# alexranaldi/CWSL_DIGI

Measured on AMD Instinct MI355X. Metric: IQ Msamples/s demod+sync per GPU; concurrent FT8 slots at real-time; % HBM roofline, higher is better.
Workload: dtype f32

## Files before the change

### cwsl_digi_amd/csrc/cwsl_gpu.hip

```cpp
#include <hip/hip_runtime.h>
#include <rccl/rccl.h>
#include <dlfcn.h>

#include <algorithm>
#include <atomic>
#include <cctype>
#include <chrono>
#include <condition_variable>
#include <cstdarg>
#include <cstdio>
#include <cstdlib>
#include <cstring>
#include <map>
#include <memory>
#include <mutex>
#include <shared_mutex>
#include <string>
#include <tuple>
#include <vector>

#ifndef CWSLG_LAB
#define CWSLG_LAB 0
#endif

// ... 123 lines not shown
    int64_t origin_abs = 0;
    bool use_priv = false;
    PhasorTable priv;
    bool trans_active = false;
    std::shared_ptr<TransWork> trans;
    int64_t pend_lo = 0;
    uint32_t pend_n = 0;
    uint64_t pend_fill0 = 0;
    bool saturated = false;
    bool have_frame = false;
    int frame_idx = 0;
    uint64_t frame_t0 = 0;
    size_t frame_valid = 0;
    bool fin_fused = false;
    FinWork fused_fin{};
    size_t i16_end = ~size_t(0);
    uint64_t cand_t0 = 0;
    SyncChannelBuffers syncbuf;
};

struct WorkBuf {
    void *h = nullptr;
    void *h_dev = nullptr;
    void *d = nullptr;
    size_t bytes = 0;
    hipEvent_t done = nullptr;
    bool in_flight = false;
};

struct TimedSpan {
    hipEvent_t a, b;
    int kind;
    unsigned gen;
};

}

using namespace cwslg;

struct cwslg_ctx {
    std::mutex mu;
    int device = 0;
    int cu_count = 256;
    int order_override = 0;
    bool exact = true;
    bool upload_by_dma = false;
    int demod_variant = 0;
    hipStream_t stream = nullptr;
    std::string last_error;
    std::mutex err_mu;
    float scale_ft = 0.90f, scale_wspr = 0.20f;
    std::vector<Receiver> rxs;
    std::vector<Channel> chans;
    std::map<uint32_t, float *> d_taps;
    std::map<uint32_t, float *> d_taps2;
    const char *demod_kernel_name = "";
    std::map<uint32_t, std::vector<float>> h_taps;
    std::map<std::tuple<uint32_t, int32_t, int, size_t>, PhasorTable> phasors;
    std::vector<decltype(phasors)::key_type> phasor_todo;
    float2 *d_sincos = nullptr;
    hipStream_t copy_stream[kCopyStreams] = {};
    hipEvent_t copy_done[kCopyStreams] = {};
    hipEvent_t demod_done = nullptr;
    bool copies_pending[kCopyStreams] = {};
    bool copy_on_main = true;
    hipStream_t fetch_stream[kFetchStreams] = {};
    hipEvent_t fetch_ev[CWSLG_NUM_GROUPS] = {};
    bool fetch_ev_valid[CWSLG_NUM_GROUPS] = {};
    unsigned fetch_rr = 0;
    std::mutex fetch_mu;
    std::condition_variable fetch_cv;
    int fetch_inflight[CWSLG_NUM_GROUPS] = {};
    std::shared_mutex life_mu;
    BatchStage batch[kBatchStages];
    std::atomic<unsigned> batch_next{0};
    std::atomic<uint64_t> push_calls_a{0}, push_host_ns_a{0};
    unsigned long long *clk_h = nullptr, *clk_dev = nullptr;
    unsigned clk_head = 0, clk_tail = 0;
    unsigned exact5_seg_cap = kExact5SegCap, exact5_seg_force = 0;
#ifndef CWSLG_FUSE_FIN_DEFAULT
#define CWSLG_FUSE_FIN_DEFAULT 1
#endif
#ifndef CWSLG_FUSE_MODE_DEFAULT
#define CWSLG_FUSE_MODE_DEFAULT 1
#endif
    int fuse_mode = CWSLG_FUSE_MODE_DEFAULT;
    bool fuse_finalize = CWSLG_FUSE_FIN_DEFAULT != 0;
    int process_min_outputs = 0;
    bool use_exact5 = true;
    unsigned stat_gen = 0;
    double clk_sum_mhz = 0.0;
    int occ_cache[3][5] = {};
    WorkBuf wb[kWorkBufs];
    int wb_next = 0;
    size_t wb_largest = 0;
    cwslg_stats stats{};
    bool timing = false;
    std::vector<TimedSpan> spans;
    std::vector<std::pair<hipEvent_t, hipEvent_t>> ev_pool;
    SyncConfig sync_cfg;
    SyncShared sync_shared;
    Ft4Tables ft4_tables{};
    bool ft4_dft_valu = false;
    LongConfig long_cfg;
    LongShared long_shared;
    hipStream_t side = nullptr;
    hipEvent_t sync2d_done = nullptr, cand_done = nullptr, sync_tail = nullptr;
    bool cand_pending = false;
    int long_variant = 0;
    int sync_variant = 0;
    cwslg_rendezvous_fn rdv_fn = nullptr;
    void *rdv_user = nullptr;
    ncclComm_t rccl_comm = nullptr;
    uint64_t *d_rdv = nullptr, *h_rdv = nullptr;
    int rccl_world = 0;
    std::atomic<uint64_t> rdv_flag{0}, rdv_flags_and{0};
    bool rdv_pending = false;
    int rdv_group = 0;
    uint64_t rdv_epoch = 0, rdv_mine = 0;
    hipEvent_t rdv_ready = nullptr;
};

namespace {

int fail(cwslg_ctx *c, int code, const char *fmt, ...)
{
    char buf[512];
    va_list ap;
    va_start(ap, fmt);
    vsnprintf(buf, sizeof(buf), fmt, ap);
    va_end(ap);
    if (c) {
        std::lock_guard<std::mutex> g(c->err_mu);
        c->last_error = buf;
    }
    return code;
}

#define HIPCHK(ctx, expr)                                                                        \
    do {                                                                                         \
        hipError_t e_ = (expr);                                                                  \
        if (e_ != hipSuccess)                                                                    \
            return fail(ctx, CWSLG_ERR_HIP, "%s failed: %s (%s:%d)", #expr, hipGetErrorString(e_), \
                        __FILE__, __LINE__);                                                     \
    } while (0)

int sync_launch(cwslg_ctx *c, const std::vector<int> &emitted);
int sync_ensure_channel(cwslg_ctx *c, Channel &ch);
int long_sync_launch(cwslg_ctx *c, const std::vector<int> &emitted);

WorkBuf *acquire_workbuf(cwslg_ctx *c, size_t bytes)
{
    WorkBuf &w = c->wb[c->wb_next];
    c->wb_next = (c->wb_next + 1) % kWorkBufs;
    if (w.in_flight) {
        hipEventSynchronize(w.done);
        w.in_flight = false;
    }
    if (w.bytes < bytes) {
        if (w.h) hipHostFree(w.h);
        if (w.d) hipFree(w.d);
        static_assert(sizeof(SyncWork) <= 128 && sizeof(ChanWork) <= 128 && sizeof(FinWork) <= 128, "per-channel descriptors");
        size_t nb = std::max<size_t>(std::max(std::max(bytes, c->wb_largest), c->chans.size() * (size_t)128), 64 << 10);
        nb = (nb + 4095) & ~size_t(4095);
        c->wb_largest = nb;
        if (hipHostMalloc(&w.h, nb, hipHostMallocDefault) != hipSuccess) return nullptr;
        if (hipHostGetDevicePointer(&w.h_dev, w.h, 0) != hipSuccess) w.h_dev = nullptr;
// ... 658 lines not shown
    }
    return CWSLG_OK;
}

int rendezvous_failed(cwslg_ctx *c, int rc)
{
    std::string inner;
    {
        std::lock_guard<std::mutex> g(c->err_mu);
        if (c->last_error.rfind("slot-boundary rendezvous:", 0) == 0) inner = c->last_error;
    }
    if (!inner.empty()) return fail(c, rc, "slot-boundary rendezvous failed (%d): %s", rc, inner.c_str() + sizeof("slot-boundary rendezvous:"));
    return fail(c, rc, "slot-boundary rendezvous failed (%d)", rc);
}

}

#include "sync_host.inc"
#include "multi_gpu.inc"
#include "longsync_host.inc"

extern "C" {

int cwslg_abi_version(void) { return CWSLG_ABI_VERSION; }

const char *cwslg_strerror(int s)
{
    switch (s) {
    case CWSLG_OK: return "ok";
    case CWSLG_ERR_RATIO: return "Fs/B must be an even integer >= 4";
    case CWSLG_ERR_BAND_LOW: return "Signal outside of band (low)";
    case CWSLG_ERR_BAND_HIGH: return "Signal outside of band (high)";
    case CWSLG_ERR_NOMEM: return "out of memory";
    case CWSLG_ERR_MODE: return "Unhandled mode";
    case CWSLG_ERR_ARG: return "invalid argument";
    case CWSLG_ERR_NO_DEVICE: return "no usable HIP device (gfx950 required; there is no CPU fallback)";
    case CWSLG_ERR_HIP: return "HIP runtime error";
    case CWSLG_ERR_NO_FRAME: return "no finalised frame";
    case CWSLG_ERR_UNSUPPORTED: return "unsupported sample rate";
    case CWSLG_ERR_BLOCK: return "block length must be a multiple of SSBD::GetInSize()";
    default: return "unknown status";
    }
}

const char *cwslg_last_error(cwslg_ctx *ctx)
{
    if (!ctx) return "";
    static thread_local std::string copy;
    std::lock_guard<std::mutex> g(ctx->err_mu);
    copy = ctx->last_error;
    return copy.c_str();
}

int cwslg_create(cwslg_ctx **out, int device_ordinal)
{
    if (!out) return CWSLG_ERR_ARG;
    *out = nullptr;
    int n = 0;
    if (hipGetDeviceCount(&n) != hipSuccess || n <= 0) return CWSLG_ERR_NO_DEVICE;
    if (device_ordinal < 0) {
        const char *lr = std::getenv("LOCAL_RANK");
        device_ordinal = lr ? std::atoi(lr) % n : 0;
    }
    if (device_ordinal >= n) return CWSLG_ERR_NO_DEVICE;
    if (hipSetDevice(device_ordinal) != hipSuccess) return CWSLG_ERR_NO_DEVICE;
    hipDeviceProp_t prop;
    if (hipGetDeviceProperties(&prop, device_ordinal) != hipSuccess) return CWSLG_ERR_NO_DEVICE;
    if (std::strncmp(prop.gcnArchName, "gfx950", 6) != 0) return CWSLG_ERR_NO_DEVICE;
    std::unique_ptr<cwslg_ctx, void (*)(cwslg_ctx *)> c(new cwslg_ctx, cwslg_destroy);
    c->device = device_ordinal;
    c->cu_count = prop.multiProcessorCount > 0 ? prop.multiProcessorCount : 256;
#if CWSLG_LAB
    if (const char *v = std::getenv("CWSLG_DEMOD_VARIANT")) c->demod_variant = std::atoi(v);
    if (c->demod_variant != 0) c->use_exact5 = false;
    if (const char *v = std::getenv("CWSLG_EXACT5_SEG")) c->exact5_seg_cap = (unsigned)std::max(4, std::atoi(v));
    if (const char *v = std::getenv("CWSLG_EXACT5_SEG_FORCE")) c->exact5_seg_force = (unsigned)std::max(4, std::atoi(v)) / 4 * 4;
    if (const char *v = std::getenv("CWSLG_UPLOAD")) c->upload_by_dma = std::strcmp(v, "dma") == 0;
    if (const char *v = std::getenv("CWSLG_FT4_DFT")) c->ft4_dft_valu = std::strcmp(v, "valu") == 0;
    if (const char *v = std::getenv("CWSLG_ITEM_ORDER")) c->order_override = std::atoi(v);
    if (const char *v = std::getenv("CWSLG_SYNC_VARIANT")) c->sync_variant = std::atoi(v);
    if (const char *v = std::getenv("CWSLG_LONG_VARIANT")) c->long_variant = std::atoi(v);
    if (const char *v = std::getenv("CWSLG_COPY_ON_MAIN")) c->copy_on_main = std::atoi(v) != 0;
    if (const char *v = std::getenv("CWSLG_FUSE_FIN")) c->fuse_finalize = std::atoi(v) != 0;
    if (const char *v = std::getenv("CWSLG_FUSE_MODE")) c->fuse_mode = std::atoi(v) == 2 ? 2 : 1;
#endif
    if (hipStreamCreateWithFlags(&c->stream, hipStreamNonBlocking) != hipSuccess) return CWSLG_ERR_HIP;
    for (int k = 0; k < kCopyStreams; ++k) {
        if (hipStreamCreateWithFlags(&c->copy_stream[k], hipStreamNonBlocking) != hipSuccess) return CWSLG_ERR_HIP;
        hipEventCreateWithFlags(&c->copy_done[k], hipEventDisableTiming);
    }
    hipEventCreateWithFlags(&c->demod_done, kOrderEvent);
    for (int k = 0; k < kFetchStreams; ++k)
        if (hipStreamCreateWithFlags(&c->fetch_stream[k], hipStreamNonBlocking) != hipSuccess) return CWSLG_ERR_HIP;
    for (hipEvent_t &e : c->fetch_ev) hipEventCreateWithFlags(&e, hipEventDisableTiming);
    if (hipStreamCreateWithFlags(&c->side, hipStreamNonBlocking) != hipSuccess) return CWSLG_ERR_HIP;
    hipEventCreateWithFlags(&c->sync2d_done, hipEventDisableTiming);
    hipEventCreateWithFlags(&c->cand_done, hipEventDisableTiming);
    hipEventCreateWithFlags(&c->sync_tail, hipEventDisableTiming);
    {
        std::vector<float2> tab(4096);
        constexpr double pi = 3.14159265358979323846;
        for (int j = 0; j < 4096; ++j)
            tab[j] = make_float2((float)std::cos(2.0 * pi * j / 4096.0), (float)std::sin(2.0 * pi * j / 4096.0));
        if (hipMalloc(&c->d_sincos, tab.size() * sizeof(float2)) != hipSuccess) return CWSLG_ERR_NOMEM;
        if (hipMemcpy(c->d_sincos, tab.data(), tab.size() * sizeof(float2), hipMemcpyHostToDevice) != hipSuccess) return CWSLG_ERR_HIP;
    }
    *out = c.release();
    return CWSLG_OK;
}

void cwslg_destroy(cwslg_ctx *c)
{
    if (!c) return;
    hipSetDevice(c->device);
    for (hipStream_t cs : c->copy_stream) if (cs) hipStreamSynchronize(cs);
    if (c->side) hipStreamSynchronize(c->side);
    if (c->stream) hipStreamSynchronize(c->stream);
    for (hipStream_t fs : c->fetch_stream) if (fs) (void)hipStreamSynchronize(fs);
    for (Channel &ch : c->chans) {
        if (ch.d_block) hipFree(ch.d_block);
        sync_free_channel(ch.syncbuf);
        if (ch.longbuf.d_block) { (void)hipFree(ch.longbuf.d_block); ch.longbuf = LongChannelBuffers(); }
        if (ch.priv.d_ckpt) { (void)hipFree(ch.priv.d_ckpt); ch.priv.d_ckpt = nullptr; }
    }
    for (Receiver &rx : c->rxs) if (rx.d_ring) hipFree(rx.d_ring);
    for (auto &kv : c->d_taps) hipFree(kv.second);
    for (auto &kv : c->d_taps2) hipFree(kv.second);
    for (auto &kv : c->phasors) if (kv.second.d_ckpt) hipFree(kv.second.d_ckpt);
    for (WorkBuf &w : c->wb) {
        if (w.h) hipHostFree(w.h);
        if (w.d) hipFree(w.d);
        if (w.done) hipEventDestroy(w.done);
    }
    drain_spans(c);
    for (auto &p : c->ev_pool) { hipEventDestroy(p.first); hipEventDestroy(p.second); }
    rccl_release(c);
    sync_free_shared(c->sync_shared);
    long_free_shared(c->long_shared);
    if (c->d_sincos) hipFree(c->d_sincos);
    if (c->clk_h) (void)hipHostFree(c->clk_h);
    for (hipStream_t fs : c->fetch_stream) if (fs) { (void)hipStreamSynchronize(fs); (void)hipStreamDestroy(fs); }
    for (hipEvent_t e : c->fetch_ev) if (e) (void)hipEventDestroy(e);
    for (BatchStage &b : c->batch) {
        if (b.h) (void)hipHostFree(b.h);
        if (b.ev) (void)hipEventDestroy(b.ev);
    }
    for (int k = 0; k < kCopyStreams; ++k) {
        if (c->copy_stream[k]) { hipStreamSynchronize(c->copy_stream[k]); hipStreamDestroy(c->copy_stream[k]); }
        if (c->copy_done[k]) hipEventDestroy(c->copy_done[k]);
    }
    if (c->demod_done) hipEventDestroy(c->demod_done);
    if (c->rdv_ready) hipEventDestroy(c->rdv_ready);
    if (c->side) { hipStreamSynchronize(c->side); hipStreamDestroy(c->side); }
    for (hipEvent_t e : {c->sync2d_done, c->cand_done, c->sync_tail}) if (e) hipEventDestroy(e);
    if (c->stream) hipStreamDestroy(c->stream);
    delete c;
}

int cwslg_set_scale_factors(cwslg_ctx *c, float ft, float wspr)
{
    if (!c) return CWSLG_ERR_ARG;
    std::lock_guard<std::mutex> g(c->mu);
    c->scale_ft = ft;
    c->scale_wspr = wspr;
    return CWSLG_OK;
}

// ... 1124 lines not shown
```

### cwsl_digi_amd/csrc/sync_host.inc

```
namespace {

int sync_ensure_shared(cwslg_ctx *c)
{
    if (c->sync_shared.d_tables) return CWSLG_OK;
    constexpr double pi = 3.14159265358979323846;
    auto w = [&](int k, double n) { return make_float2((float)std::cos(2.0 * pi * k / n), (float)(-std::sin(2.0 * pi * k / n))); };
    auto half = [](float2 v) { return make_float2(0.5f * v.x, 0.5f * v.y); };
    auto same = [](float a, float b) { return std::memcmp(&a, &b, 4) == 0; };
    for (int k = 1; k <= 4; ++k)
        if (!same(w(k, 9.0).x, small_wr<9>(k)) || !same(w(k, 9.0).y, small_wi<9>(k)))
            return fail(c, CWSLG_ERR_HIP, "sync tables: W_9^%d computed on this host differs from the kernels' constants", k);
    for (int k = 1; k <= 2; ++k)
        if (!same(w(k, 5.0).x, w5_r(k)) || !same(w(k, 5.0).y, w5_i(k)))
            return fail(c, CWSLG_ERR_HIP, "sync tables: W_5^%d computed on this host differs from the kernels' constants", k);
    if (!same((float)(-std::sin(2.0 * pi / 3.0)), W3_S))
        return fail(c, CWSLG_ERR_HIP, "sync tables: sin(2 pi / 3) computed on this host differs from the kernels' constant");
    std::vector<float2> t;
    t.reserve(1920 + 64 + 1921 + 1152 + 1153);
    const float fac = 1.0f / 300.0f;
    for (int k = 0; k < 1920; ++k) { const float2 v = (k == 0) ? make_float2(1.f, 0.f) : w(k, 1920.0); t.push_back(make_float2(fac * v.x, fac * v.y)); }
    for (int k = 0; k < 64; ++k) t.push_back(w(k, 128.0));
    for (int k = 0; k <= 1920; ++k) t.push_back(half(k == 0 ? make_float2(1.f, 0.f) : w(k, 3840.0)));
    t[1920] = make_float2(1.f, 0.f); t[1920 + 32] = make_float2(0.f, -1.f);
    const size_t ft8_count = t.size();
// ... 124 lines not shown
int sync_launch(cwslg_ctx *c, const std::vector<int> &emitted)
{
    int rc = sync_ensure_shared(c);
    if (rc) return rc;
    const SyncConfig &cfg = c->sync_cfg;
    std::vector<SyncWork> works8, works4;
    std::vector<Ft4Work> works4c;
    for (int id : emitted) {
        Channel &ch = c->chans[id];
        if (!ch.sync_ft8 && !ch.sync_ft4) continue;
        rc = sync_ensure_channel(c, ch);
        if (rc) return rc;
        SyncWork w{};
        w.frame = ch.d_i16;
        w.spectra = ch.syncbuf.d_spectra;
        w.red = ch.syncbuf.d_red; w.red2 = ch.syncbuf.d_red2;
        w.jpeak = ch.syncbuf.d_jpeak; w.jpeak2 = ch.syncbuf.d_jpeak2;
        w.cand = ch.syncbuf.d_cand; w.ncand = ch.syncbuf.d_ncand;
        if (ch.fin_fused) { w.fin = ch.fused_fin; ch.fin_fused = false; }
        (ch.sync_ft8 ? works8 : works4).push_back(w);
        ch.cand_t0 = ch.frame_t0;
        if (ch.sync_ft4 && cfg.ft4_coherent) {
            if ((rc = ft4c_ensure_tables(c)) != CWSLG_OK || (rc = ft4c_ensure_channel(c, ch)) != CWSLG_OK) return rc;
            Ft4Work f{};
            f.frame = ch.d_i16; f.y = ch.syncbuf.d_y; f.cx = ch.syncbuf.d_cx;
            f.cand = ch.syncbuf.d_cand; f.ncand = ch.syncbuf.d_ncand;
            f.rec = (Ft4Rec *)ch.syncbuf.d_rec; f.nrec = ch.syncbuf.d_nrec; f.cd_dbg = ch.syncbuf.d_cd_dbg;
            works4c.push_back(f);
        }
    }
    if (works8.empty() && works4.empty()) return CWSLG_OK;
    const size_t n8 = works8.size(), n4 = works4.size();
    WorkBuf *wb = acquire_workbuf(c, (n8 + n4) * sizeof(SyncWork));
    if (!wb) return fail(c, CWSLG_ERR_NOMEM, "work buffer allocation failed");
    if (n8) std::memcpy(wb->h, works8.data(), n8 * sizeof(SyncWork));
    if (n4) std::memcpy((SyncWork *)wb->h + n8, works4.data(), n4 * sizeof(SyncWork));
    HIPCHK(c, upload_workbuf(c, wb, (n8 + n4) * sizeof(SyncWork)));
    WorkBuf *wb4 = nullptr;
    if (!works4c.empty()) {
        wb4 = acquire_workbuf(c, works4c.size() * sizeof(Ft4Work));
        if (!wb4) return fail(c, CWSLG_ERR_NOMEM, "work buffer allocation failed");
        std::memcpy(wb4->h, works4c.data(), works4c.size() * sizeof(Ft4Work));
        HIPCHK(c, upload_workbuf(c, wb4, works4c.size() * sizeof(Ft4Work)));
    }
    hipEvent_t ea, eb;
    const bool chain_async = n8 && !n4 && (c->sync_variant & 32);
    const bool cand_async = n8 && (c->sync_variant & 8) && !chain_async;
    if (n8 && c->cand_pending) {
        HIPCHK(c, hipStreamWaitEvent(c->stream, c->cand_done, 0));
        c->cand_pending = false;
    }
    hipStream_t s8 = c->stream;
    if (chain_async) {
        s8 = c->side;
        HIPCHK(c, hipEventRecord(c->sync2d_done, c->stream));
        HIPCHK(c, hipStreamWaitEvent(c->side, c->sync2d_done, 0));
        span_begin_on(c, 2, c->side, &ea, &eb);
    } else {
        span_begin(c, 2, &ea, &eb);
    }
    if (n8) {
        const SyncWork *d8 = (const SyncWork *)wb->d;
        const unsigned nbands = (unsigned)((cfg.ib - cfg.ia + 1 + SYNC_BAND - 1) / SYNC_BAND);
#if CWSLG_LAB
        if (c->sync_variant & 2)
            hipLaunchKernelGGL((symbol_spectra_kernel<15, FT8_NSPS, FT8_NSTEP, false>), dim3(FT8_NHSYM, (unsigned)n8), dim3(256), 0,
                               s8, d8, c->sync_shared.t, cfg.nbins);
        else
#endif
        {
        hipEvent_t pa = nullptr, pb = nullptr;
        if (s8 == c->stream) span_begin(c, 3, &pa, &pb);
        const int jper8 = spectra_jper(FT8_NHSYM, n8);
        bool fused8 = works8[0].fin.frame != nullptr;
        for (const SyncWork &sw : works8) if ((sw.fin.frame != nullptr) != fused8) return fail(c, CWSLG_ERR_ARG, "mixed fused / separate finalise in one launch");
        const dim3 g8((FT8_NHSYM + jper8 - 1) / jper8, (unsigned)n8);
        if (!fused8) {
#if CWSLG_LAB || !CWSLG_FUSE_FIN_DEFAULT
            hipLaunchKernelGGL((symbol_spectra_v2_kernel<15, FT8_NSPS, FT8_NSTEP, false, 0>), g8, dim3(256), 0, s8, d8, c->sync_shared.t, cfg.nbins, FT8_NHSYM, jper8);
#else
            return fail(c, CWSLG_ERR_ARG, "FT8 frame reached the sync stage without its finalise");
#endif
        }
#if CWSLG_LAB || CWSLG_FUSE_MODE_DEFAULT == 2
        else if (c->fuse_mode == 2)
            hipLaunchKernelGGL((symbol_spectra_v2_kernel<15, FT8_NSPS, FT8_NSTEP, false, 2>), g8, dim3(256), 0, s8, d8, c->sync_shared.t, cfg.nbins, FT8_NHSYM, jper8);
#endif
        else
            hipLaunchKernelGGL((symbol_spectra_v2_kernel<15, FT8_NSPS, FT8_NSTEP, false, 1>), g8, dim3(256), 0, s8, d8, c->sync_shared.t, cfg.nbins, FT8_NHSYM, jper8);
        span_end(c, pb);
        }
        const bool per_channel = n8 >= (size_t)2 * (size_t)c->cu_count;
#if CWSLG_LAB
        if (!(c->sync_variant & (1 | 64 | 128))) {
#endif
        hipEvent_t qa = nullptr, qb = nullptr;
        if (s8 == c->stream) span_begin(c, 4, &qa, &qb);
        if (per_channel) {
            hipLaunchKernelGGL(ft8_sync_chan_kernel, dim3((unsigned)n8), dim3(SYNCC_NT), 0, s8, d8, cfg.ia, cfg.ib, cfg.nbins, cfg.syncmin, cfg.max_cand, cfg.order);
        } else {
            hipLaunchKernelGGL(ft8_sync2d_v3_kernel, dim3(nbands, (unsigned)n8), dim3(SYNC2D_NT), 0, s8, d8, cfg.ia, cfg.ib, cfg.nbins);
            hipLaunchKernelGGL(ft8_candidates_kernel<1024>, dim3((unsigned)n8), dim3(1024), 0, s8, d8, cfg.ia, cfg.ib, cfg.syncmin, cfg.max_cand, cfg.order);
        }
        span_end(c, qb);
#if CWSLG_LAB
        } else {
        if (c->sync_variant & 1)
            hipLaunchKernelGGL(ft8_sync2d_kernel, dim3(nbands, (unsigned)n8), dim3(SYNC2D_NT), 0, s8, d8, cfg.ia, cfg.ib, cfg.nbins);
        else if (c->sync_variant & 64)
            hipLaunchKernelGGL(ft8_sync2d_v2_kernel, dim3(nbands, (unsigned)n8), dim3(SYNC2D_NT), 0, s8, d8, cfg.ia, cfg.ib, cfg.nbins);
        else
            hipLaunchKernelGGL(ft8_sync2d_v3_kernel, dim3(nbands, (unsigned)n8), dim3(SYNC2D_NT), 0, s8, d8, cfg.ia, cfg.ib, cfg.nbins);
        hipStream_t cs = s8;
        hipEvent_t sa = nullptr, sb = nullptr;
        if (cand_async) {
            cs = c->side;
            HIPCHK(c, hipEventRecord(c->sync2d_done, c->stream));
            HIPCHK(c, hipStreamWaitEvent(c->side, c->sync2d_done, 0));
            span_begin_on(c, 2, c->side, &sa, &sb);
        }
        if (c->sync_variant & 4)
            hipLaunchKernelGGL(ft8_candidates_kernel<256>, dim3((unsigned)n8), dim3(256), 0, cs, d8, cfg.ia, cfg.ib,
                               cfg.syncmin, cfg.max_cand, cfg.order);
        else
            hipLaunchKernelGGL(ft8_candidates_kernel<1024>, dim3((unsigned)n8), dim3(1024), 0, cs, d8, cfg.ia, cfg.ib,
                               cfg.syncmin, cfg.max_cand, cfg.order);
        if (cand_async) {
            if (sb) hipEventRecord(sb, c->side);
            HIPCHK(c, hipEventRecord(c->cand_done, c->side));
            c->cand_pending = true;
        }
        }
#endif
    }
    if (n4) {
        const SyncWork *d4 = (const SyncWork *)wb->d + n8;
        const float df4 = 12000.0f / (float)FT4_NFFT1;
        int nfa = (int)((float)cfg.f_lo_hz / df4), nfb = (int)((float)cfg.f_hi_hz / df4);
        nfa = std::max(nfa, (int)std::lround(200.0f / df4));
        nfb = std::min(nfb, (int)std::lround(4910.0f / df4));
        const int jper4 = spectra_jper(FT4_NHSYM, n4);
#if CWSLG_LAB
        if (c->sync_variant & 2)
            hipLaunchKernelGGL((symbol_spectra_kernel<9, FT4_NFFT1, FT4_NSTEP, true>), dim3(FT4_NHSYM, (unsigned)n4), dim3(256), 0,
                               c->stream, d4, c->sync_shared.t4, FT4_ROW);
        else
#endif
        hipLaunchKernelGGL((symbol_spectra_v2_kernel<9, FT4_NFFT1, FT4_NSTEP, true>), dim3((FT4_NHSYM + jper4 - 1) / jper4, (unsigned)n4), dim3(256), 0,
                           c->stream, d4, c->sync_shared.t4, FT4_ROW, FT4_NHSYM, jper4);
        hipLaunchKernelGGL(ft4_candidates_kernel, dim3((unsigned)n4), dim3(256), 0, c->stream, d4, nfa, nfb,
                           c->sync_cfg.syncmin_ft4, cfg.max_cand, cfg.order);
        if (c->sync_cfg.ft4_coherent) {
            const Ft4Work *f4 = (const Ft4Work *)wb4->d;
#if CWSLG_LAB
            if (c->ft4_dft_valu)
                hipLaunchKernelGGL(ft4_dft567_kernel, dim3((F4C_NA + 4 * F4C_CPT - 1) / (4 * F4C_CPT), (unsigned)n4), dim3(256), 0, c->stream, f4, c->ft4_tables);
            else
#endif
            hipLaunchKernelGGL(ft4_dft567_mfma_kernel, dim3(9, (unsigned)n4), dim3(256), 0, c->stream, f4, c->ft4_tables);
            hipLaunchKernelGGL(ft4_fft64_unpack_kernel, dim3(284, (unsigned)n4), dim3(64), 0, c->stream, f4, c->ft4_tables);
            hipLaunchKernelGGL(ft4_refine_kernel, dim3((unsigned)cfg.max_cand, (unsigned)n4), dim3(256), 0, c->stream, f4, c->ft4_tables, cfg.max_cand);
        }
    }
    if (chain_async) {
        if (eb) hipEventRecord(eb, c->side);
        HIPCHK(c, hipEventRecord(c->cand_done, c->side));
        c->cand_pending = true;
        HIPCHK(c, hipGetLastError());
        HIPCHK(c, hipEventRecord(wb->done, c->side));
        wb->in_flight = true;
        c->stats.sync_launches++;
        return CWSLG_OK;
// ... 175 lines not shown
```

### cwsl_digi_amd/csrc/sync_kernels.hpp

```cpp
#pragma once
#include <hip/hip_runtime.h>
#include <stdint.h>

namespace cwslg {

constexpr int FT8_NSPS = 1920, FT8_NSTEP = 480, FT8_NHSYM = 372, FT8_NH1 = 1920, FT8_JZ = 62, FT8_NMAX = 180000;
constexpr int FT4_NFFT1 = 2304, FT4_NSTEP = 576, FT4_NHSYM = 122, FT4_NH1 = 1152, FT4_NMAX = 72576;
constexpr int FT4_ROW = 1168;
constexpr int SYNC_BAND = 32;
constexpr int SYNC_MAXCAND_CAP = 600;
constexpr int SYNC_MAXPRE = 1000;

struct SyncConfig {
    bool enabled = false;
    float syncmin = 1.5f;
    float syncmin_ft4 = 1.2f;
    bool ft4_coherent = true;
    int max_cand = 200;
    int order = 0;
    int f_lo_hz = 200, f_hi_hz = 3000;
    int ia = 64, ib = 960, nbins = 976;
};

struct SyncTables {
// ... 391 lines not shown
#define CWSLG_SPEC_TIGHT 1
#endif
#ifndef CWSLG_PLANE_NT
#define CWSLG_PLANE_NT 0
#endif
__device__ __forceinline__ void plane_store(CWSLG_GLOBAL v4f *p, v4f v)
{
    if (CWSLG_PLANE_NT & 1) __builtin_nontemporal_store(v, p); else *p = v;
}
__device__ __forceinline__ v4f plane_load4(const CWSLG_GLOBAL v4f *p)
{
    return (CWSLG_PLANE_NT & 2) ? __builtin_nontemporal_load(p) : *p;
}
__device__ __forceinline__ float plane_load1(const CWSLG_GLOBAL float *p)
{
    return (CWSLG_PLANE_NT & 2) ? __builtin_nontemporal_load(p) : *p;
}
inline int spectra_jper(int nsteps, size_t channels)
{
    for (int jper : {62, 31}) if (channels * (size_t)((nsteps + jper - 1) / jper) >= 3072) return jper;
    return 12;
}
#if defined(CWSLG_STAMP) && defined(CWSLG_STAMP_SPEC)
#define PSTAMP(slot)                                                                                                               \
    do {                                                                                                                           \
        const unsigned wg_ = blockIdx.y * gridDim.x + blockIdx.x;                                                                  \
        if (j == j0 + (jper >> 1) && (tid_ & 63) == 0 && wg_ < 16384) {                                                                     \
            unsigned long long t_;                                                                                                 \
            asm volatile("s_memtime %0\n\ts_waitcnt lgkmcnt(0)" : "=s"(t_)::"memory");                                             \
            g_stamps[32 * wg_ + 8 * (tid_ >> 6) + (slot)] = t_;                                                                    \
        }                                                                                                                          \
    } while (0)
#else
#define PSTAMP(slot) do { } while (0)
#endif
struct SpectraFin {
    const CWSLG_GLOBAL float *frame;
    CWSLG_GLOBAL int16_t *out;
    unsigned nv, s_end;
    float factor;
};
__device__ __forceinline__ unsigned fin_pack2(float x0, float x1, float factor)
{
    const float s0 = x0 * factor, s1 = x1 * factor;
    const float b0 = s0 + 0.5f, b1 = s1 + 0.5f;
    const int q0 = (int)b0, q1 = (int)b1;
    return ((unsigned)q0 & 0xFFFFu) | ((unsigned)q1 << 16);
}
__device__ __forceinline__ void spectra_finalize_range(const SpectraFin &F, unsigned s0, unsigned s1)
{
    typedef unsigned v4u __attribute__((ext_vector_type(4)));
    constexpr int NC = 4;
    for (unsigned base = s0 + threadIdx.x * 8u; base < s1; base += 256u * 8u * (unsigned)NC) {
        v4f a[NC], b[NC];
#pragma unroll
        for (int c = 0; c < NC; ++c) {
            const unsigned i0 = base + (unsigned)c * (256u * 8u);
            if (i0 + 8 <= F.nv && i0 < s1) {
                a[c] = *reinterpret_cast<const CWSLG_GLOBAL v4f *>(F.frame + i0);
                b[c] = *reinterpret_cast<const CWSLG_GLOBAL v4f *>(F.frame + i0 + 4);
            } else {
                float v[8];
#pragma unroll
                for (int k = 0; k < 8; ++k) v[k] = (i0 + k < F.nv && i0 < s1) ? F.frame[i0 + k] : 0.0f;
                a[c] = v4f{v[0], v[1], v[2], v[3]};
                b[c] = v4f{v[4], v[5], v[6], v[7]};
            }
        }
#pragma unroll
        for (int c = 0; c < NC; ++c) {
            const unsigned i0 = base + (unsigned)c * (256u * 8u);
            if (i0 >= s1) break;
            v4u pk;
            pk.x = fin_pack2(a[c].x, a[c].y, F.factor); pk.y = fin_pack2(a[c].z, a[c].w, F.factor);
            pk.z = fin_pack2(b[c].x, b[c].y, F.factor); pk.w = fin_pack2(b[c].z, b[c].w, F.factor);
            *reinterpret_cast<CWSLG_GLOBAL v4u *>(F.out + i0) = pk;
        }
    }
}

template <int NA, int NIN, int STEP, bool WINDOW, int FMODE = 0>
__global__ __launch_bounds__(256, CWSLG_SPEC_WAVES) void symbol_spectra_v2_kernel(const SyncWork *__restrict__ works, SyncTables tb, int nbins, int nsteps, int jper)
{
    static_assert(FMODE == 0 || (!WINDOW && NIN == 4 * STEP && STEP == 480), "the fused forms are FT8's");
    constexpr int NZ = NA * 128;
    constexpr int NPACK = NIN / 2;
    constexpr int NGRP = NA * 16;
    constexpr int AMAX = (NPACK + 127) / 128;
    constexpr int NH = NA / 2;
    constexpr int NITEM = (NH + 1) * 64, IPT = (NITEM + 255) / 256;
    static_assert(NGRP <= 256, "geometry");
    __shared__ __attribute__((aligned(16))) float s_pw[NIN + 32];
    __shared__ float2 s_y[NA][SY_PITCH];
    __shared__ float2 s_w128[64];
    constexpr int RING = NPACK + STEP / 2;
    __shared__ unsigned s_ring[FMODE == 2 ? 2 * RING : 1];
    const SyncWork *w = works + blockIdx.y;
    const int j0 = blockIdx.x * jper;
    const int jend = min(j0 + jper, nsteps);
    const int tid_ = threadIdx.x;
    const int b_ = tid_ & 127;
    const float fac = 1.0f / 300.0f;
    const CWSLG_GLOBAL unsigned *d32 = as_global(reinterpret_cast<const unsigned *>(w->frame)) + b_;
    float *const plane = w->spectra;
    const bool fuse = FMODE != 0;
    SpectraFin F{};
    v2f cv = {0.0f, 0.0f};
    unsigned fin_i = ~0u;
    unsigned fin_lim = 0u;
    constexpr int LOOK = 3;
    unsigned ring_rd = 0u, ring_wr = 0u;
    if (fuse) {
        const FinWork &f = w->fin;
        F.frame = as_global(f.frame); F.out = as_global_rw(f.out); F.nv = f.n_valid;
        const unsigned flen = f.frame_len;
        const float peak = __uint_as_float(*as_global(f.peak));
        float factor = 32767.0f / (peak + 1.0f);
        factor = factor * f.scale;
        F.factor = factor;
        if (blockIdx.x == 0 && tid_ == 0) {
            if (f.peak_next) *as_global_rw(f.peak_next) = 0u;
            if (f.factor_out) *as_global_rw(f.factor_out) = factor;
        }
        const unsigned cover = min((unsigned)(STEP * (nsteps - 1) + NIN), flen), tail_end = min(max(f.tail_end, cover), flen);
        if (tail_end > cover) {
            const unsigned per = ((tail_end - cover + gridDim.x - 1) / gridDim.x + 7u) & ~7u;
            spectra_finalize_range(F, min(cover + per * blockIdx.x, tail_end), min(cover + per * (blockIdx.x + 1), tail_end));
        }
        if constexpr (FMODE == 1) {
            F.s_end = min(((unsigned)(STEP * (jend - 1) + NIN) + 63u) & ~63u, flen);
            const unsigned e0 = min(((unsigned)(STEP * (j0 + LOOK - 1) + NIN) + 63u) & ~63u, F.s_end);
            spectra_finalize_range(F, (unsigned)(STEP * j0) & ~63u, e0);
            __builtin_amdgcn_s_waitcnt(0x0F70);
            __syncthreads();
            fin_lim = min(F.nv & ~1u, F.s_end);
            fin_i = e0 + 2u * (unsigned)tid_;
        } else {
            F.s_end = min((unsigned)(STEP * (jend - 1) + NIN), flen);
            fin_lim = min(F.nv & ~1u, F.s_end);
            const unsigned p0 = (unsigned)(STEP / 2) * (unsigned)j0;
            for (unsigned k = (unsigned)tid_; k < (unsigned)NPACK; k += 256u) {
                const unsigned i = 2u * (p0 + k);
                v2f p = {0.0f, 0.0f};
                if (i < fin_lim) p = *reinterpret_cast<const CWSLG_GLOBAL v2f *>(F.frame + i);
                const v2f bi = p * F.factor + 0.5f;
                const unsigned word = __builtin_amdgcn_perm((unsigned)(int)bi.y, (unsigned)(int)bi.x, 0x05040100u);
                if (i < F.s_end) *reinterpret_cast<CWSLG_GLOBAL unsigned *>(F.out + i) = word;
                const unsigned pos = (p0 + k) % (unsigned)RING;
                s_ring[pos] = word; s_ring[pos + RING] = word;
            }
            __syncthreads();
            fin_i = tid_ < STEP / 2 ? (unsigned)(STEP * j0 + NIN) + 2u * (unsigned)tid_ : 0x40000000u;
            ring_rd = (p0 + (unsigned)b_) % (unsigned)RING;
            ring_wr = (p0 + (unsigned)NPACK + (unsigned)tid_) % (unsigned)RING;
        }
        if (fin_i < fin_lim) cv = *reinterpret_cast<const CWSLG_GLOBAL v2f *>(F.frame + fin_i);
    }
    unsigned raw[AMAX];
    if constexpr (FMODE != 2) {
#pragma unroll
        for (int a = 0; a < AMAX; ++a) raw[a] = (128 * a + b_ < NPACK) ? d32[(STEP / 2) * j0 + 128 * a] : 0u;
    } else {
#pragma unroll
        for (int a = 0; a < AMAX; ++a) raw[a] = s_ring[ring_rd + 128 * a];
        ring_rd += (unsigned)(STEP / 2); if (ring_rd >= (unsigned)RING) ring_rd -= (unsigned)RING;
    }
    float2 wn[WINDOW ? AMAX : 1];
    if (WINDOW) {
#pragma unroll
        for (int a = 0; a < AMAX; ++a) {
            const int m = 128 * a + b_;
            wn[WINDOW ? a : 0] = *reinterpret_cast<const float2 *>(tb.win + 2 * ((m < NPACK) ? m : 0));
        }
    }
    Stage1Tw<NA> tw1;
    if (tid_ < 128) stage1_load_tw<0, NA>(tb.w1920, b_, tw1);
    else stage1_load_tw<1, NA>(tb.w1920, b_, tw1);
    const bool sparse = nbins >= NA * 64 && nbins <= NA * 64 + 32 && NH == 7;
    constexpr unsigned PW_DUMMY = 4u * (NIN + 31);
    float2 w3[IPT][2];
#ifndef CWSLG_SPEC_UNHOIST
#define CWSLG_SPEC_UNHOIST 0
#endif
    struct ItemAddr { unsigned au1[IPT], au2[IPT], aw1[IPT], aw2[IPT], ap1[IPT], ap2[IPT], aB[8]; bool iskip[IPT], izero[IPT]; };
    auto item_addr = [&](int tidx, ItemAddr &A, int (&K1o)[IPT], int (&K2o)[IPT]) {
#pragma unroll
    for (int i = 0; i < IPT; ++i) {
        const int it = tidx + 256 * i;
        int r = it >> 6, q = it & 63, kind = 0;
        bool skip = it >= NITEM || (r == 0 && q > 32);
        int Kup = 0;
        if (sparse && i == 0 && r == 0 && q > 32) {
            Kup = NA * 64 - 32 + q;
            const int d = Kup - NA * 64, a = d / NA, rem = d % NA;
            if (rem <= NH) { kind = 2; r = rem; q = a; }
            else { kind = 3; r = NA - rem; q = 63 - a; }
            skip = Kup >= nbins;
        }
        const int r2 = (r == 0) ? 0 : NA - r;
        const int k2 = (r == 0) ? ((64 - q) & 63) : 63 - q;
        A.izero[i] = r == 0 && q == 0 && kind == 0;
        if (sparse && A.izero[i]) kind = 1;
        A.iskip[i] = skip;
        const int rr = skip ? 0 : r, rr2 = skip ? 0 : r2;
        static_assert((SY_PITCH * 8) % 128 == 0, "row pitch");
        A.au1[i] = 8u * (unsigned)(rr * SY_PITCH + sy_col(q));
        A.au2[i] = 8u * (unsigned)(rr2 * SY_PITCH + sy_col(k2));
        A.aw1[i] = 8u * (unsigned)q; A.aw2[i] = 8u * (unsigned)k2;
        int K1 = NA * q + r, K2 = NA * k2 + r2;
        unsigned p1 = 4u * (unsigned)K1, p2 = 4u * (unsigned)K2;
        if (kind == 1) { K2 = NA * 64; p2 = (K2 < nbins) ? 4u * (unsigned)K2 : PW_DUMMY; }
        if (kind >= 2) { K1 = Kup; p1 = 4u * (unsigned)Kup; K2 = nbins; p2 = PW_DUMMY; }
        A.ap1[i] = p1 | ((unsigned)kind << 16); A.ap2[i] = p2;
        K1o[i] = (!skip && K1 < nbins) ? K1 : -1; K2o[i] = (!skip && K2 < nbins) ? K2 : -1;
    }
    {
        const int c = tidx >> 4, g = tidx & 15, blk = g >> 3, r = g & 7;
#pragma unroll
        for (int q = 0; q < 8; ++q) A.aB[q] = 8u * (unsigned)((tidx < NGRP ? c : 0) * SY_PITCH + sy_col(64 * blk + r + 8 * q));
    }
    };
    ItemAddr IA0;
    {
        int K1o[IPT], K2o[IPT];
        item_addr(tid_, IA0, K1o, K2o);
#pragma unroll
        for (int i = 0; i < IPT; ++i) {
            w3[i][0] = K1o[i] >= 0 ? tb.w3840[K1o[i]] : make_float2(0.f, 0.f);
            w3[i][1] = K2o[i] >= 0 ? tb.w3840[K2o[i]] : make_float2(0.f, 0.f);
        }
    }
    const bool wave0_ = __builtin_amdgcn_readfirstlane(tid_ >> 6) == 0;
    if (tid_ >= 64 && tid_ < 128) s_w128[tid_ - 64] = tb.w128[tid_ - 64];
    __builtin_amdgcn_s_waitcnt(0x0F70);

    for (int j = j0; j < jend; ++j) {
    int t = tid_;
    asm volatile("" : "+v"(t));
    const int tid = t, b = t & 127;
    ItemAddr IAj;
    int k1j[IPT], k2j[IPT];
    if (CWSLG_SPEC_UNHOIST) item_addr(tid, IAj, k1j, k2j);
    const ItemAddr &IA = CWSLG_SPEC_UNHOIST ? IAj : IA0;
    char *const sy_bytes = reinterpret_cast<char *>(&s_y[0][0]);
    const char *const w128_bytes = reinterpret_cast<const char *>(&s_w128[0]);
    char *const pw_bytes = reinterpret_cast<char *>(&s_pw[0]);
    PSTAMP(0);
    float2 z[AMAX];
#pragma unroll
    for (int a = 0; a < AMAX; ++a) {
        const bool live = 128 * a + b < NPACK;
        float lo = (float)(short)(raw[a] & 0xFFFFu), hi = (float)(short)(raw[a] >> 16);
        if (NA != 15) { lo = fac * lo; hi = fac * hi; }
        if (WINDOW) { lo = lo * wn[WINDOW ? a : 0].x; hi = hi * wn[WINDOW ? a : 0].y; }
        z[a] = live ? make_float2(lo, hi) : make_float2(0.f, 0.f);
    }
#ifndef CWSLG_SPEC_LOADS_FIRST
#define CWSLG_SPEC_LOADS_FIRST 0
#endif
#ifndef CWSLG_FUSE_STORE_NT
#define CWSLG_FUSE_STORE_NT 0
#endif
    auto store_prev_row = [&]() {
#ifdef CWSLG_SPEC_DIAG_NOSTORE
        if (j > j0 && nbins < 0) {
#else
        if (j > j0) {
#endif
            CWSLG_GLOBAL v4f *out4 = reinterpret_cast<CWSLG_GLOBAL v4f *>(as_global_rw(CWSLG_SPEC_HOISTPTR ? plane : w->spectra) + (size_t)(j - 1) * nbins);
            if (NA == 15) { if (tid >= 128) for (int k4 = tid - 128; 4 * k4 < nbins; k4 += 128) plane_store(out4 + k4, *reinterpret_cast<const v4f *>(s_pw + 4 * k4)); }
            else for (int k4 = tid; 4 * k4 < nbins; k4 += 256) plane_store(out4 + k4, *reinterpret_cast<const v4f *>(s_pw + 4 * k4));
        }
    };
    if (!CWSLG_SPEC_LOADS_FIRST) store_prev_row();
    if (fuse) {
        const v2f sc = cv * F.factor;
        const v2f bi = sc + 0.5f;
        const int q0 = (int)bi.x, q1 = (int)bi.y;
        const unsigned word = __builtin_amdgcn_perm((unsigned)q1, (unsigned)q0, 0x05040100u);
        if (fin_i < F.s_end) {
            if (CWSLG_FUSE_STORE_NT) __builtin_nontemporal_store(word, reinterpret_cast<CWSLG_GLOBAL unsigned *>(F.out + fin_i));
            else *reinterpret_cast<CWSLG_GLOBAL unsigned *>(F.out + fin_i) = word;
            if constexpr (FMODE == 2) { s_ring[ring_wr] = word; s_ring[ring_wr + RING] = word; }
        }
        if constexpr (FMODE == 2) {
            fin_i += (unsigned)STEP;
            ring_wr += (unsigned)(STEP / 2); if (ring_wr >= (unsigned)RING) ring_wr -= (unsigned)RING;
        } else {
            fin_i += 512u;
        }
        cv = v2f{0.0f, 0.0f};
        if (fin_i < fin_lim) cv = *reinterpret_cast<const CWSLG_GLOBAL v2f *>(F.frame + fin_i);
    }
    {
        const int jn = CWSLG_SPEC_TIGHT ? min(j + 1, jend - 1) : j + 1;
        if constexpr (FMODE != 2) {
        if (CWSLG_SPEC_TIGHT || j + 1 < jend)
#pragma unroll
        for (int a = 0; a < AMAX; ++a) raw[a] = (128 * a + b < NPACK) ? d32[(STEP / 2) * jn + 128 * a] : 0u;
        }
    }
    if (CWSLG_SPEC_LOADS_FIRST) store_prev_row();

    if (tid < 128) spectra_stage1_regs<0, NA, AMAX>(z, s_y, tw1, b);
    else spectra_stage1_regs<1, NA, AMAX>(z, s_y, tw1, b);
    PSTAMP(1);
    lds_barrier();
    PSTAMP(2);
    if constexpr (FMODE == 2) {
#pragma unroll
        for (int a = 0; a < AMAX; ++a) raw[a] = s_ring[ring_rd + 128 * a];
        ring_rd += (unsigned)(STEP / 2); if (ring_rd >= (unsigned)RING) ring_rd -= (unsigned)RING;
    }

#ifndef CWSLG_SPEC_MERGE_AB
#define CWSLG_SPEC_MERGE_AB 1
#endif
    const bool inAB = tid < NGRP;
    if (CWSLG_SPEC_MERGE_AB ? inAB : true) {
    {
        const int c = tid >> 4, g = tid & 15;
        const int gb = (int)(__brev((unsigned)g) >> 28);
        float2 e[8];
        if (CWSLG_SPEC_MERGE_AB || inAB) {
            const char *const pa = sy_bytes + 8u * (unsigned)(c * SY_PITCH + gb);
#pragma unroll
            for (int k = 0; k < 8; ++k) {
                const int k3 = ((k & 1) << 2) | (k & 2) | ((k >> 2) & 1);
                e[k] = CWSLG_SPEC_TIGHT ? *reinterpret_cast<const float2 *>(pa + 128 * k3) : s_y[c][16 * k3 + gb];
            }
        }
        __builtin_amdgcn_fence(__ATOMIC_RELEASE, "wavefront");
        __builtin_amdgcn_wave_barrier();
        __builtin_amdgcn_fence(__ATOMIC_ACQUIRE, "wavefront");
        if (CWSLG_SPEC_MERGE_AB || inAB) {
            bfly_one(e[0], e[1]); bfly_one(e[2], e[3]); bfly_one(e[4], e[5]); bfly_one(e[6], e[7]);
            bfly_one(e[0], e[2]); bfly_mj(e[1], e[3]); bfly_one(e[4], e[6]); bfly_mj(e[5], e[7]);
            bfly_one(e[0], e[4]); bfly(e[1], e[5], s_w128[16]); bfly_mj(e[2], e[6]); bfly(e[3], e[7], s_w128[48]);
            const unsigned a0 = 8u * (unsigned)(c * SY_PITCH + sy_col(8 * g));
#pragma unroll
            for (int k = 0; k < 8; ++k) {
                if (CWSLG_SPEC_TIGHT) *reinterpret_cast<float2 *>(sy_bytes + (a0 ^ (8u * k))) = e[k];
                else s_y[c][sy_col(8 * g + k)] = e[k];
            }
        }
    }
    __builtin_amdgcn_fence(__ATOMIC_RELEASE, "wavefront");
    __builtin_amdgcn_wave_barrier();
    __builtin_amdgcn_fence(__ATOMIC_ACQUIRE, "wavefront");
    PSTAMP(3);
    if (CWSLG_SPEC_MERGE_AB || inAB) {
        const int r = tid & 7;
        float2 e[8];
#pragma unroll
        for (int q = 0; q < 8; ++q) e[q] = *reinterpret_cast<const float2 *>(sy_bytes + IA.aB[q]);
        {
            const float2 w0 = s_w128[r * 8];
            bfly(e[0], e[1], w0); bfly(e[2], e[3], w0); bfly(e[4], e[5], w0); bfly(e[6], e[7], w0);
        }
        {
            const float2 w0 = s_w128[r * 4], w1 = s_w128[(r + 8) * 4];
            bfly(e[0], e[2], w0); bfly(e[1], e[3], w1); bfly(e[4], e[6], w0); bfly(e[5], e[7], w1);
        }
        {
            bfly(e[0], e[4], s_w128[r * 2]); bfly(e[1], e[5], s_w128[(r + 8) * 2]);
            bfly(e[2], e[6], s_w128[(r + 16) * 2]); bfly(e[3], e[7], s_w128[(r + 24) * 2]);
        }
#pragma unroll
        for (int q = 0; q < 8; ++q) *reinterpret_cast<float2 *>(sy_bytes + IA.aB[q]) = e[q];
    }
    }
    PSTAMP(4);
    lds_barrier();
    PSTAMP(5);

    float2 w3j[IPT][2];
    if (CWSLG_SPEC_UNHOIST) {
#pragma unroll
        for (int i = 0; i < IPT; ++i) {
            w3j[i][0] = k1j[i] >= 0 ? tb.w3840[k1j[i]] : make_float2(0.f, 0.f);
            w3j[i][1] = k2j[i] >= 0 ? tb.w3840[k2j[i]] : make_float2(0.f, 0.f);
        }
    }
    const float2 (&w3u)[IPT][2] = CWSLG_SPEC_UNHOIST ? w3j : w3;
#pragma unroll
    for (int i = 0; i < IPT; ++i) {
        if (IA.iskip[i]) continue;
        float2 u1 = *reinterpret_cast<const float2 *>(sy_bytes + IA.au1[i]), v1 = *reinterpret_cast<const float2 *>(sy_bytes + (IA.au1[i] ^ 64u) + 512);
        float2 u2 = *reinterpret_cast<const float2 *>(sy_bytes + IA.au2[i]), v2 = *reinterpret_cast<const float2 *>(sy_bytes + (IA.au2[i] ^ 64u) + 512);
        bfly(u1, v1, *reinterpret_cast<const float2 *>(w128_bytes + IA.aw1[i]));
        bfly(u2, v2, *reinterpret_cast<const float2 *>(w128_bytes + IA.aw2[i]));
        if (sparse) {
            float2 A1 = u1, B1 = v2, A2 = u2;
            unsigned p1 = IA.ap1[i];
            if (i == 0 && wave0_) {
                const unsigned kind = p1 >> 16;
// ... 1078 lines not shown
```

Before: 316,600.

## Add fused mode 3 reading float frames directly in symbol spectra kernel

Adds a new fused-finalise form (mode 3) and makes it the default. The FT8 symbol-spectra kernel now loads the float frame directly, quantises it in registers to build its FFT input, and writes the packed int16 words for each step's new samples. It replaces the old ring-buffer mode 2 and the separate lagging finalise stream of mode 1. This removes a dependency on previously written int16 data and an LDS ring, at the cost of loading twice as many bytes per window (float2 instead of packed shorts) and redundant quantisation across overlapping windows.

```diff
diff --git a/cwsl_digi_amd/csrc/cwsl_gpu.hip b/cwsl_digi_amd/csrc/cwsl_gpu.hip
--- a/cwsl_digi_amd/csrc/cwsl_gpu.hip
+++ b/cwsl_digi_amd/csrc/cwsl_gpu.hip
@@ -229,7 +229,7 @@
 #define CWSLG_FUSE_FIN_DEFAULT 1
 #endif
 #ifndef CWSLG_FUSE_MODE_DEFAULT
-#define CWSLG_FUSE_MODE_DEFAULT 1
+#define CWSLG_FUSE_MODE_DEFAULT 3
 #endif
     int fuse_mode = CWSLG_FUSE_MODE_DEFAULT;
     bool fuse_finalize = CWSLG_FUSE_FIN_DEFAULT != 0;
@@ -1054,7 +1054,7 @@
     if (const char *v = std::getenv("CWSLG_LONG_VARIANT")) c->long_variant = std::atoi(v);
     if (const char *v = std::getenv("CWSLG_COPY_ON_MAIN")) c->copy_on_main = std::atoi(v) != 0;
     if (const char *v = std::getenv("CWSLG_FUSE_FIN")) c->fuse_finalize = std::atoi(v) != 0;
-    if (const char *v = std::getenv("CWSLG_FUSE_MODE")) c->fuse_mode = std::atoi(v) == 2 ? 2 : 1;
+    if (const char *v = std::getenv("CWSLG_FUSE_MODE")) c->fuse_mode = std::atoi(v) == 1 ? 1 : 3;
 #endif
     if (hipStreamCreateWithFlags(&c->stream, hipStreamNonBlocking) != hipSuccess) return CWSLG_ERR_HIP;
     for (int k = 0; k < kCopyStreams; ++k) {
diff --git a/cwsl_digi_amd/csrc/sync_host.inc b/cwsl_digi_amd/csrc/sync_host.inc
--- a/cwsl_digi_amd/csrc/sync_host.inc
+++ b/cwsl_digi_amd/csrc/sync_host.inc
@@ -230,12 +230,12 @@
             return fail(c, CWSLG_ERR_ARG, "FT8 frame reached the sync stage without its finalise");
 #endif
         }
-#if CWSLG_LAB || CWSLG_FUSE_MODE_DEFAULT == 2
-        else if (c->fuse_mode == 2)
-            hipLaunchKernelGGL((symbol_spectra_v2_kernel<15, FT8_NSPS, FT8_NSTEP, false, 2>), g8, dim3(256), 0, s8, d8, c->sync_shared.t, cfg.nbins, FT8_NHSYM, jper8);
+#if CWSLG_LAB || CWSLG_FUSE_MODE_DEFAULT == 1
+        else if (c->fuse_mode == 1)
+            hipLaunchKernelGGL((symbol_spectra_v2_kernel<15, FT8_NSPS, FT8_NSTEP, false, 1>), g8, dim3(256), 0, s8, d8, c->sync_shared.t, cfg.nbins, FT8_NHSYM, jper8);
 #endif
         else
-            hipLaunchKernelGGL((symbol_spectra_v2_kernel<15, FT8_NSPS, FT8_NSTEP, false, 1>), g8, dim3(256), 0, s8, d8, c->sync_shared.t, cfg.nbins, FT8_NHSYM, jper8);
+            hipLaunchKernelGGL((symbol_spectra_v2_kernel<15, FT8_NSPS, FT8_NSTEP, false, 3>), g8, dim3(256), 0, s8, d8, c->sync_shared.t, cfg.nbins, FT8_NHSYM, jper8);
         span_end(c, pb);
         }
         const bool per_channel = n8 >= (size_t)2 * (size_t)c->cu_count;
diff --git a/cwsl_digi_amd/csrc/sync_kernels.hpp b/cwsl_digi_amd/csrc/sync_kernels.hpp
--- a/cwsl_digi_amd/csrc/sync_kernels.hpp
+++ b/cwsl_digi_amd/csrc/sync_kernels.hpp
@@ -497,6 +497,7 @@
 template <int NA, int NIN, int STEP, bool WINDOW, int FMODE = 0>
 __global__ __launch_bounds__(256, CWSLG_SPEC_WAVES) void symbol_spectra_v2_kernel(const SyncWork *__restrict__ works, SyncTables tb, int nbins, int nsteps, int jper)
 {
+    static_assert(FMODE == 0 || FMODE == 1 || FMODE == 3, "forms");
     static_assert(FMODE == 0 || (!WINDOW && NIN == 4 * STEP && STEP == 480), "the fused forms are FT8's");
     constexpr int NZ = NA * 128;
     constexpr int NPACK = NIN / 2;
@@ -508,8 +509,6 @@
     __shared__ __attribute__((aligned(16))) float s_pw[NIN + 32];
     __shared__ float2 s_y[NA][SY_PITCH];
     __shared__ float2 s_w128[64];
-    constexpr int RING = NPACK + STEP / 2;
-    __shared__ unsigned s_ring[FMODE == 2 ? 2 * RING : 1];
     const SyncWork *w = works + blockIdx.y;
     const int j0 = blockIdx.x * jper;
     const int jend = min(j0 + jper, nsteps);
@@ -524,7 +523,9 @@
     unsigned fin_i = ~0u;
     unsigned fin_lim = 0u;
     constexpr int LOOK = 3;
-    unsigned ring_rd = 0u, ring_wr = 0u;
+    const CWSLG_GLOBAL v2f *f2 = nullptr;
+    CWSLG_GLOBAL unsigned *o32 = nullptr;
+    unsigned lim2 = 0u;
     if (fuse) {
         const FinWork &f = w->fin;
         F.frame = as_global(f.frame); F.out = as_global_rw(f.out); F.nv = f.n_valid;
@@ -551,34 +552,32 @@
             fin_lim = min(F.nv & ~1u, F.s_end);
             fin_i = e0 + 2u * (unsigned)tid_;
         } else {
-            F.s_end = min((unsigned)(STEP * (jend - 1) + NIN), flen);
-            fin_lim = min(F.nv & ~1u, F.s_end);
-            const unsigned p0 = (unsigned)(STEP / 2) * (unsigned)j0;
-            for (unsigned k = (unsigned)tid_; k < (unsigned)NPACK; k += 256u) {
-                const unsigned i = 2u * (p0 + k);
-                v2f p = {0.0f, 0.0f};
-                if (i < fin_lim) p = *reinterpret_cast<const CWSLG_GLOBAL v2f *>(F.frame + i);
-                const v2f bi = p * F.factor + 0.5f;
-                const unsigned word = __builtin_amdgcn_perm((unsigned)(int)bi.y, (unsigned)(int)bi.x, 0x05040100u);
-                if (i < F.s_end) *reinterpret_cast<CWSLG_GLOBAL unsigned *>(F.out + i) = word;
-                const unsigned pos = (p0 + k) % (unsigned)RING;
-                s_ring[pos] = word; s_ring[pos + RING] = word;
-            }
-            __syncthreads();
-            fin_i = tid_ < STEP / 2 ? (unsigned)(STEP * j0 + NIN) + 2u * (unsigned)tid_ : 0x40000000u;
-            ring_rd = (p0 + (unsigned)b_) % (unsigned)RING;
-            ring_wr = (p0 + (unsigned)NPACK + (unsigned)tid_) % (unsigned)RING;
-        }
+            f2 = reinterpret_cast<const CWSLG_GLOBAL v2f *>(F.frame) + b_;
+            o32 = reinterpret_cast<CWSLG_GLOBAL unsigned *>(F.out) + tid_;
+            lim2 = min(F.nv & ~1u, cover) >> 1;
+        }
+        if constexpr (FMODE == 1)
         if (fin_i < fin_lim) cv = *reinterpret_cast<const CWSLG_GLOBAL v2f *>(F.frame + fin_i);
     }
-    unsigned raw[AMAX];
-    if constexpr (FMODE != 2) {
+    unsigned raw[FMODE == 3 ? 1 : AMAX];
+    v2f rawf[FMODE == 3 ? AMAX : 1];
+    auto load_window_f = [&](int jn, int bb) {
+        const unsigned p0 = (unsigned)(STEP / 2) * (unsigned)jn;
+        const CWSLG_GLOBAL v2f *src = f2 + p0;
+        if (p0 + (unsigned)NPACK <= lim2) {
+#pragma unroll
+            for (int a = 0; a < AMAX; ++a) rawf[FMODE == 3 ? a : 0] = (128 * a + bb < NPACK) ? src[128 * a] : v2f{0.0f, 0.0f};
+        } else {
+#pragma unroll
+            for (int a = 0; a < AMAX; ++a)
+                rawf[FMODE == 3 ? a : 0] = (128 * a + bb < NPACK && p0 + (unsigned)(128 * a + bb) < lim2) ? src[128 * a] : v2f{0.0f, 0.0f};
+        }
+    };
+    if constexpr (FMODE == 3) {
+        load_window_f(j0, b_);
+    } else {
 #pragma unroll
         for (int a = 0; a < AMAX; ++a) raw[a] = (128 * a + b_ < NPACK) ? d32[(STEP / 2) * j0 + 128 * a] : 0u;
-    } else {
-#pragma unroll
-        for (int a = 0; a < AMAX; ++a) raw[a] = s_ring[ring_rd + 128 * a];
-        ring_rd += (unsigned)(STEP / 2); if (ring_rd >= (unsigned)RING) ring_rd -= (unsigned)RING;
     }
     float2 wn[WINDOW ? AMAX : 1];
     if (WINDOW) {
@@ -664,11 +663,21 @@
     float2 z[AMAX];
 #pragma unroll
     for (int a = 0; a < AMAX; ++a) {
+        if constexpr (FMODE == 3) {
+            const v2f sc = rawf[a] * F.factor;
+            const v2f bi = sc + 0.5f;
+            z[a] = make_float2((float)(short)(int)bi.x, (float)(short)(int)bi.y);
+            continue;
+        }
         const bool live = 128 * a + b < NPACK;
-        float lo = (float)(short)(raw[a] & 0xFFFFu), hi = (float)(short)(raw[a] >> 16);
+        float lo = (float)(short)(raw[FMODE == 3 ? 0 : a] & 0xFFFFu), hi = (float)(short)(raw[FMODE == 3 ? 0 : a] >> 16);
         if (NA != 15) { lo = fac * lo; hi = fac * hi; }
         if (WINDOW) { lo = lo * wn[WINDOW ? a : 0].x; hi = hi * wn[WINDOW ? a : 0].y; }
         z[a] = live ? make_float2(lo, hi) : make_float2(0.f, 0.f);
+    }
+    if constexpr (FMODE == 3) {
+#pragma unroll
+        for (int a = 0; a < AMAX; ++a) asm volatile("" : "+v"(z[a].x), "+v"(z[a].y));
     }
 #ifndef CWSLG_SPEC_LOADS_FIRST
 #define CWSLG_SPEC_LOADS_FIRST 0
@@ -688,7 +697,7 @@
         }
     };
     if (!CWSLG_SPEC_LOADS_FIRST) store_prev_row();
-    if (fuse) {
+    if constexpr (FMODE == 1) {
         const v2f sc = cv * F.factor;
         const v2f bi = sc + 0.5f;
         const int q0 = (int)bi.x, q1 = (int)bi.y;
@@ -696,20 +705,30 @@
         if (fin_i < F.s_end) {
             if (CWSLG_FUSE_STORE_NT) __builtin_nontemporal_store(word, reinterpret_cast<CWSLG_GLOBAL unsigned *>(F.out + fin_i));
             else *reinterpret_cast<CWSLG_GLOBAL unsigned *>(F.out + fin_i) = word;
-            if constexpr (FMODE == 2) { s_ring[ring_wr] = word; s_ring[ring_wr + RING] = word; }
-        }
-        if constexpr (FMODE == 2) {
-            fin_i += (unsigned)STEP;
-            ring_wr += (unsigned)(STEP / 2); if (ring_wr >= (unsigned)RING) ring_wr -= (unsigned)RING;
-        } else {
-            fin_i += 512u;
-        }
+        }
+        fin_i += 512u;
         cv = v2f{0.0f, 0.0f};
         if (fin_i < fin_lim) cv = *reinterpret_cast<const CWSLG_GLOBAL v2f *>(F.frame + fin_i);
     }
+    if constexpr (FMODE == 3) {
+        const bool upper = tid >= 128;
+        auto word_of = [&](int k) {
+            const float2 x = upper ? z[2 * k + 1] : z[2 * k];
+            return __builtin_amdgcn_perm((unsigned)(int)x.y, (unsigned)(int)x.x, 0x05040100u);
+        };
+        CWSLG_GLOBAL unsigned *const dst = o32 + (unsigned)(STEP / 2) * (unsigned)j;
+        if (j + 1 < nsteps) {
+            if (tid < STEP / 2) dst[0] = word_of(0);
+        } else {
+#pragma unroll
+            for (int k = 0; k < 4; ++k) if (256 * k + tid < NPACK) dst[256 * k] = word_of(k);
+        }
+    }
     {
         const int jn = CWSLG_SPEC_TIGHT ? min(j + 1, jend - 1) : j + 1;
-        if constexpr (FMODE != 2) {
+        if constexpr (FMODE == 3) {
+            load_window_f(jn, b);
+        } else {
         if (CWSLG_SPEC_TIGHT || j + 1 < jend)
 #pragma unroll
         for (int a = 0; a < AMAX; ++a) raw[a] = (128 * a + b < NPACK) ? d32[(STEP / 2) * jn + 128 * a] : 0u;
@@ -722,11 +741,6 @@
     PSTAMP(1);
     lds_barrier();
     PSTAMP(2);
-    if constexpr (FMODE == 2) {
-#pragma unroll
-        for (int a = 0; a < AMAX; ++a) raw[a] = s_ring[ring_rd + 128 * a];
-        ring_rd += (unsigned)(STEP / 2); if (ring_rd >= (unsigned)RING) ring_rd -= (unsigned)RING;
-    }
 
 #ifndef CWSLG_SPEC_MERGE_AB
 #define CWSLG_SPEC_MERGE_AB 1
```

After: 314,300. About the same (-0.7%).
